# JohannesBuchner/UltraNest

Measured on AMD Instinct MI355X. Metric: proposal-points filtered/sec (MLFriends.inside) + region-rebuild ms, N=4000 d=50, higher is better.
Workload: dtype f64; 1 GPU; C5: N=4000 live points, d=50, P=1e6 proposals/step/GPU drawn uniformly inside the wrapping ellipsoid (set E), AffineLayer, 30 bootstraps; one step = MLFriends.inside on a batch resident in HBM; the timed loop visits 3 distinct batches in turn; n_live=4000, d=50, bootstraps=30, parallelism=proposal rows sharded over 1 GPU(s), region replicated

## Files before the change

ultranest_amd/csrc/mlf_filter.hpp:

```cpp
#pragma once
#include "mlf_common.hpp"
#include "mlf_prep4.hpp"

#define MLF_FILTER_MAXD 128

constexpr int kFilterMaxSplit = 16;

namespace mlf {

struct FilterArgs {
  const void *refF;
  const void *qF;
  const float *tlo, *thi;
  int ntiles32;
  long long ngroups;
  long long nq;
  int *best;
  unsigned long long *list;
  unsigned seg_cap;
  unsigned *seg_count;
  unsigned *counters;
  int tile0, tile1;
  const int *qmap;
  const unsigned *ngroups_dev;
  const unsigned *nslots_dev;
  int append;
  void *cq;
  float *ctlo, *cthi;
  int *cmap;
  unsigned *ccount;
  unsigned ccap;
  const uint8_t *route;
  long long seg_first_extra, seg_extra;
  int split;
  RecheckWArgs rw;
};
struct MinArgs {
  const void *refF;
  int ntiles32;
  int tile0, tile1;
  const void *qF;
  const float *tlo, *thi;
  const int *qmap;
  const int *qmin;
  long long ngroups;
  const unsigned *nslots_dev;
  long long nq;
  int *best;
  void *cq;
  float *ctlo, *cthi;
  int *cmap;
  int *cmin;
  unsigned *ccount;
  unsigned ccap;
  int last;
  unsigned long long *stamps;
  unsigned stamp_block;
};
constexpr unsigned kUncertainListCap = 4096;
struct UncertainArgs {
  const void *refF;
  int ntiles32;
  const void *qF;
  const float *thi;
  const int *qmap;
  const unsigned *nslots_dev;
  const double *pts;
  int d, dp;
  const double *lay_ctr;
  const double *T8;
  int ldt8;
  const double *refR;
  int n;
  double r2;
  int *best;
  unsigned *counters;
  unsigned *seg_count;
  EllExactArgs ell;
  unsigned nsweepblk;
};
hipError_t launch_sweep_min(int ks, int qw, const MinArgs &a, hipStream_t s);
hipError_t launch_uncertain(int ks, const UncertainArgs &a, hipStream_t s);
long long uncertain_blocks();
__host__ __device__ constexpr unsigned uncertain_stamp_base() { return 256u; }

struct MidArgs {
  const double *pts;
  long long np;
  int d, dp, ks;
  const void *LtF;
  const float *y0;
  const void *TtF;
  const double *lay_ctr;
  Prep4Consts c;
  const double *stats;
  double r2;
  const double *ell_ctr, *ell_L, *ell_A;
  double ell_eps_scale, enlarge;
  int chol_ok;
  const void *refF;
  int ntiles32;
  const double *refR;
  int n;
  const double *T64;
  unsigned long long *rec;
  unsigned long long *meta;
  unsigned *arrive;
  uint8_t *mask;
  uint8_t *route;
  unsigned *scan_flag;
  unsigned *counters;
  unsigned *stamps;
};
#define MLF_FOR_EACH_DP_MID(X)                                                                \
  X(2) X(4) X(6) X(8) X(10) X(12) X(14) X(16) X(18) X(20) X(22) X(24) X(26) X(28) X(30) X(32) \
  X(36) X(40) X(44) X(48) X(50) X(52) X(56)
bool mid_usable(int dp);
int mid_range_quads(long long ngroups, int ntiles32);
hipError_t launch_inside_mid(const MidArgs &a, int ny, hipStream_t s);

struct FusedArgs {
  Prep4Args p;
  const void *refF;
  int ntiles32;
  int tile0, tile1;
  void *cq;
  float *ctlo, *cthi;
  int *cmap, *cmin;
  unsigned *ccount;
  unsigned ccap;
  unsigned long long *stamps;
  unsigned stamp_block;
  unsigned variant;
};
bool fused_usable(int dp);
hipError_t launch_prep_sweep(const FusedArgs &a, hipStream_t s, int waves = 8);

void launch_phase_finish(void *cq, float *ctlo, float *cthi, int *cmap, unsigned *ccount, unsigned *ngroups_dst,
                         int ks, hipStream_t s);

struct RecheckArgs {
  const unsigned long long *list;
  unsigned seg_cap;
  const unsigned *seg_count;
  const double *refR;
  int n, d, dp;
  const double *q;
  long long ldq, ldk, nq;
  double r2;
  int *best;
};

void launch_ref_stats(const double *refR, int n, int d, int dp, double *stats, double *scratch, hipStream_t s,
                      unsigned long long *keys = nullptr);
void launch_quant_refs(const double *refR, int n, int npad32, int d, int dp, int ks,
                       const double *stats, void *refF, hipStream_t s, void *refFm = nullptr, const int *perm = nullptr,
                       double *rows_out = nullptr, int nrows_out = 0);
void launch_ref_rank(const unsigned long long *keys, int n, int *perm, hipStream_t s);
void launch_quant_queries(const double *q, long long ldq, long long nq, long long nqpad, int d_src, int d, int ks,
                          const double *stats, double r2, const uint8_t *gate, void *qF, float *tlo,
                          float *thi, uint8_t *route, int *best, unsigned *counters, hipStream_t s);
hipError_t launch_filter(int ks, const FilterArgs &a, bool first, hipStream_t s, int narrow = 0);
hipError_t launch_sweep(int ks, int qw, const FilterArgs &a, hipStream_t s);
int filter_groups_per_wave(int ks, int narrow);
void launch_recheck(const RecheckArgs &a, long long nwaves, hipStream_t s);
long long filter_wave_count(int ks, long long ngroups, int narrow = 0);
int filter_tile_split(int ks, long long ngroups, int ntiles, int target_waves = 2048);
void launch_filter_finalize(const uint8_t *route, const int *best, const unsigned *counters, long long nq,
                            uint8_t *out_mask, long long *out_idx, uint8_t *exact_gate, hipStream_t s,
                            unsigned *reset_word = nullptr);
void launch_route_gate(const uint8_t *route, const unsigned *counters, long long nq, int which,
                       uint8_t *gate, hipStream_t s);

}
```

ultranest_amd/csrc/mlf_sweepmin.hip:

```cpp
#include "mlf_filter.hpp"
#include "mlf_dpp_dev.hpp"
#include "mlf_filter_dev.hpp"
#include "mlf_recheck_dev.hpp"

#include <math.h>

namespace mlf {

typedef __attribute__((ext_vector_type(8))) _Float16 half8;
typedef __attribute__((ext_vector_type(16))) float float16v;
typedef __attribute__((ext_vector_type(4))) unsigned uint4v;

namespace {

__device__ __forceinline__ int min3i(int a, int b, int c) {
  const int m = a < b ? a : b;
  return m < c ? m : c;
}

constexpr int kPosInf = 0x7f800000;

template <int KS>
__device__ __forceinline__ void load_tile(half8 (&A)[KS], __amdgpu_buffer_rsrc_t rsrc, int voff, int soff) {
#pragma unroll
  for (int s = 0; s < KS; ++s) {
    union { uint4v u; half8 h; } c;
    c.u = __builtin_amdgcn_raw_buffer_load_b128(rsrc, voff, soff + s * 1024, 0);
    A[s] = c.h;
  }
}

__device__ __forceinline__ int tree_min(const float16v &c, int run) {
  const int m0 = min3i(__float_as_int(c[0]), __float_as_int(c[1]), __float_as_int(c[2]));
  const int m1 = min3i(__float_as_int(c[3]), __float_as_int(c[4]), __float_as_int(c[5]));
  const int m2 = min3i(__float_as_int(c[6]), __float_as_int(c[7]), __float_as_int(c[8]));
  const int m3 = min3i(__float_as_int(c[9]), __float_as_int(c[10]), __float_as_int(c[11]));
  const int m4 = min3i(__float_as_int(c[12]), __float_as_int(c[13]), __float_as_int(c[14]));
  return min3i(min3i(m0, m1, m2), min3i(m3, m4, __float_as_int(c[15])), run);
}

template <int I, int NM, int NV>
__device__ __forceinline__ void pin_step() {
  if constexpr (I < NM) {
    __builtin_amdgcn_sched_group_barrier(0x008, 1, 0);
    __builtin_amdgcn_sched_group_barrier(0x002, (NV * (I + 1)) / NM - (NV * I) / NM, 0);
    pin_step<I + 1, NM, NV>();
  }
}

__host__ __device__ constexpr int uncertain_row_stride(int d) { return d; }

__device__ __forceinline__ int uni(int v) { return __builtin_amdgcn_readfirstlane(v); }
__device__ __forceinline__ long long uni(long long v) {
  const unsigned lo = (unsigned)__builtin_amdgcn_readfirstlane((int)(unsigned)v);
  const unsigned hi = (unsigned)__builtin_amdgcn_readfirstlane((int)(unsigned)((unsigned long long)v >> 32));
  return (long long)(((unsigned long long)hi << 32) | lo);
}
template <class T>
__device__ __forceinline__ T *uni(T *p) {
  return reinterpret_cast<T *>(static_cast<uintptr_t>(uni((long long)reinterpret_cast<uintptr_t>(p))));
}

constexpr int min_waves(int ks, int qw, int pf) {
  const int need = 16 * qw + 4 * ks * qw + 4 * ks * (pf + 1) + 40;
  return (qw <= 2 && ks * qw <= 8) ? 4 : (need <= 128 ? 4 : (need <= 168 ? 3 : 2));
}

constexpr long long kSweepMinSetGrid = 1024;

}

template <int KS, int QW, int PF>
__global__ __launch_bounds__(256) __attribute__((amdgpu_waves_per_eu(min_waves(KS, QW, PF)))) void k_sweep_min(MinArgs a) {
  const int lane = threadIdx.x & 63;
  const long long nslots = a.nslots_dev ? (long long)*a.nslots_dev : -1;
  const long long ngroups = nslots >= 0 ? (nslots + 31) / 32 : a.ngroups;
  __shared__ unsigned wg_keep[4], wg_base;
  bool stamp_on = a.stamps != nullptr && blockIdx.x == a.stamp_block && threadIdx.x < 64;
  auto stamp = [&](int k) __attribute__((always_inline)) {
    if (stamp_on) {
      const unsigned long long t = __builtin_readcyclecounter();
      if (lane == 0) a.stamps[k] = t;
    }
  };
  stamp(0);
  auto stamp_rt = [&](int k) __attribute__((always_inline)) {
    if (a.stamps != nullptr && threadIdx.x == 0) {
      if (blockIdx.x == 0) a.stamps[8 + k] = __builtin_amdgcn_s_memrealtime();
      if (blockIdx.x == a.stamp_block) a.stamps[10 + k] = __builtin_amdgcn_s_memrealtime();
    }
  };
  stamp_rt(0);
  for (unsigned bidx = blockIdx.x, pass = 0;; bidx += gridDim.x, ++pass) {
  if ((long long)bidx * (4 * QW) >= ngroups) break;
  if (pass) __syncthreads();
  const long long wave = (long long)bidx * 4 + (threadIdx.x >> 6);
  const long long g0 = wave * QW;
  if (g0 >= ngroups) {
    if (lane == 0) wg_keep[threadIdx.x >> 6] = 0u;
    __syncthreads();
    __syncthreads();
    continue;
  }

  const half8 *qF = reinterpret_cast<const half8 *>(a.qF);
  half8 bq[QW][KS];
  float tlo[QW], thi[QW];
  int run[QW], qnum[QW];
#pragma unroll
  for (int g = 0; g < QW; ++g) {
    const long long grp = (g0 + g < ngroups) ? g0 + g : ngroups - 1;
#pragma unroll
    for (int s = 0; s < KS; ++s) bq[g][s] = qF[((size_t)grp * KS + s) * 64 + lane];
    const long long qi = grp * 32 + (lane & 31);
    const bool have = g0 + g < ngroups && (nslots < 0 || qi < nslots);
    tlo[g] = have ? a.tlo[qi] : -1.0f;
    thi[g] = have ? a.thi[qi] : -1.0f;
    if (!have) {
#pragma unroll
      for (int s = 0; s < KS; ++s) bq[g][s] = (half8){0, 0, 0, 0, 0, 0, 0, 0};
    }
    run[g] = (a.qmin && have && lane < 32) ? a.qmin[qi] : kPosInf;
    qnum[g] = have ? (a.qmap ? a.qmap[qi] : (int)qi) : -1;
  }

  const int ntl = a.tile1 - a.tile0;
  const int tstart = a.tile0 + (int)(((long long)bidx * 37) % ntl);
  constexpr int kTileBytes = KS * 1024;
  const __amdgpu_buffer_rsrc_t rsrc =
      __builtin_amdgcn_make_buffer_rsrc(const_cast<void *>(a.refF), 0, a.ntiles32 * kTileBytes, 0x00020000);
  const int voff = lane * 16;
  const int off_begin = a.tile0 * kTileBytes, off_end = a.tile1 * kTileBytes;

  float16v acc[QW];
  auto mm = [&](const half8(&A)[KS], int ga, int gb) __attribute__((always_inline)) {
#pragma unroll
    for (int s = 0; s < KS; ++s) {
      const float16v z = {0.f, 0.f, 0.f, 0.f, 0.f, 0.f, 0.f, 0.f, 0.f, 0.f, 0.f, 0.f, 0.f, 0.f, 0.f, 0.f};
      acc[ga] = __builtin_amdgcn_mfma_f32_32x32x16_f16(A[s], bq[ga][s], s == 0 ? z : acc[ga], 0, 0, 0);
      if (gb >= 0) acc[gb] = __builtin_amdgcn_mfma_f32_32x32x16_f16(A[s], bq[gb][s], s == 0 ? z : acc[gb], 0, 0, 0);
    }
  };
  auto next_off = [&](int off) __attribute__((always_inline)) {
    const int n = off + kTileBytes;
    return n == off_end ? off_begin : n;
  };
  auto tile = [&](const half8(&A)[KS]) __attribute__((always_inline)) {
    constexpr int NP = (QW + 1) / 2;
#pragma unroll
    for (int p = 0; p <= NP; ++p) {
      __builtin_amdgcn_sched_barrier(0);
      if (p < NP) mm(A, 2 * p, (2 * p + 1 < QW) ? 2 * p + 1 : -1);
      if (p > 0) {
#pragma unroll
        for (int g = 2 * (p - 1); g < 2 * p && g < QW; ++g) run[g] = tree_min(acc[g], run[g]);
      }
      if (NP == 2 && p == 1) pin_step<0, (QW == 4 ? 2 : 1) * KS, 16>();
    }
    __builtin_amdgcn_sched_barrier(0);
  };

  half8 A0[KS], A1[KS];
  if (PF == 2) {
    half8 A2[KS];
    int o0 = tstart * kTileBytes, o1 = next_off(o0), o2 = next_off(o1);
    load_tile<KS>(A0, rsrc, voff, o0);
    __builtin_amdgcn_sched_barrier(0);
    load_tile<KS>(A1, rsrc, voff, o1);
    __builtin_amdgcn_sched_barrier(0);
    stamp(1);
    for (int it = 0; it < ntl; it += 3) {
      load_tile<KS>(A2, rsrc, voff, o2);
      tile(A0);
      if (it == 0) stamp(2);
      if (it + 1 >= ntl) break;
      o0 = next_off(o2);
      load_tile<KS>(A0, rsrc, voff, o0);
      tile(A1);
      if (it + 2 >= ntl) break;
      o1 = next_off(o0);
      load_tile<KS>(A1, rsrc, voff, o1);
      tile(A2);
      o2 = next_off(o1);
    }
  } else {
    int off = tstart * kTileBytes;
    load_tile<KS>(A0, rsrc, voff, off);
    for (int it = 0; it < ntl; it += 2) {
      const int offn = next_off(off);
      load_tile<KS>(A1, rsrc, voff, offn);
      tile(A0);
      if (it + 1 >= ntl) break;
      off = next_off(offn);
      load_tile<KS>(A0, rsrc, voff, off);
      tile(A1);
    }
  }

  stamp(3);
  unsigned keepm[QW];
  int qid[QW], qmn[QW];
#pragma unroll
  for (int g = 0; g < QW; ++g) {
    keepm[g] = 0u;
    qid[g] = -1;
    qmn[g] = kPosInf;
    if (g0 + g >= ngroups) continue;
    const long long qi = qnum[g];
    const int m = half_min32(run[g]);
    const float mf = __int_as_float(m);
    const bool valid = qi >= 0 && qi < a.nq && thi[g] > 0.0f;
    const bool hit = valid && mf <= tlo[g];
    if (lane < 32 && hit) a.best[qi] = 0;
    const bool keep = valid && !hit && (a.last ? mf <= thi[g] : true);
    keepm[g] = (unsigned)__ballot(keep);
    qid[g] = (int)qi;
    qmn[g] = m;
  }
  unsigned total = 0;
#pragma unroll
  for (int g = 0; g < QW; ++g) total += (unsigned)__popc(keepm[g]);
  if (lane == 0) wg_keep[threadIdx.x >> 6] = total;
  stamp(4);
  __syncthreads();
  stamp(5);
  if (threadIdx.x == 0) {
    const unsigned all = wg_keep[0] + wg_keep[1] + wg_keep[2] + wg_keep[3];
    wg_base = all ? atomicAdd(a.ccount, all) : 0u;
  }
  __syncthreads();
  stamp(6);
  if (total != 0u) {
    unsigned base = wg_base;
    for (int w = 0; w < (int)(threadIdx.x >> 6); ++w) base += wg_keep[w];
    base = (unsigned)__builtin_amdgcn_readfirstlane((int)base);
    uint4 *dst = reinterpret_cast<uint4 *>(a.cq);
    const unsigned row = (unsigned)(lane & 31);
#pragma unroll
    for (int g = 0; g < QW; ++g) {
      if ((keepm[g] >> row) & 1u) {
        const unsigned rank = base + (unsigned)__popc(keepm[g] & ((1u << row) - 1u));
        const size_t gd = rank >> 5;
        const unsigned rd = (rank & 31u) + (unsigned)(lane & 32);
        if (rank < a.ccap) {
#pragma unroll
          for (int s = 0; s < KS; ++s) {
            union { half8 h; uint4 u; } cv;
            cv.h = bq[g][s];
            dst[(gd * KS + s) * 64 + rd] = cv.u;
          }
        }
        if (lane < 32 && rank < a.ccap) {
          a.ctlo[rank] = tlo[g];
          a.cthi[rank] = thi[g];
          a.cmap[rank] = qid[g];
          if (a.cmin) a.cmin[rank] = qmn[g];
        }
      }
      base += (unsigned)__popc(keepm[g]);
    }
  }
  stamp(7);
  if (stamp_on || (pass == 0 && blockIdx.x == 0)) stamp_rt(1);
  stamp_on = false;
  }
}

template <class T>
using lds_t = __attribute__((address_space(3))) T;
template <class T>
__device__ __forceinline__ lds_t<T> *lds_ptr(T *p) {
  return (lds_t<T> *)p;
}
template <class T>
__device__ __forceinline__ const lds_t<T> *lds_ptr(const T *p) {
  return (const lds_t<T> *)p;
}

template <int KS>
__device__ __attribute__((noinline)) void uncertain_sweep(const void *refF_, int ntiles32_, const void *qF_, const float *thi_, long long set_,
                                                          long long ngroups_, long long nslots_, unsigned *plist_, unsigned *lcount_,
                                                          int wv_, int lane) {
  constexpr int QW = 4;
  lds_t<unsigned> *plist = lds_ptr(plist_);
  lds_t<unsigned> *lcount = lds_ptr(lcount_);
  const void *refF = uni(refF_);
  const int ntiles32 = uni(ntiles32_), wv = uni(wv_);
  const long long set = uni(set_), ngroups = uni(ngroups_), nslots = uni(nslots_);
  qF_ = uni(qF_);
  thi_ = uni(thi_);
  typedef __attribute__((address_space(1))) const half8 ghalf8;
  typedef __attribute__((address_space(1))) const float gfloat;
  ghalf8 *qF = (ghalf8 *)qF_;
  gfloat *thig = (gfloat *)thi_;
  constexpr int kTileBytes = KS * 1024;
  const __amdgpu_buffer_rsrc_t rsrc =
      __builtin_amdgcn_make_buffer_rsrc(const_cast<void *>(refF), 0, ntiles32 * kTileBytes, 0x00020000);
  const int voff = lane * 16;
  const int rowbase = 4 * (lane >> 5);
  const long long g0 = set * QW;
  half8 bq[QW][KS];
  float thi[QW];
#pragma unroll
  for (int g = 0; g < QW; ++g) {
    const long long grp = (g0 + g < ngroups) ? g0 + g : ngroups - 1;
#pragma unroll
    for (int s = 0; s < KS; ++s) bq[g][s] = qF[((size_t)grp * KS + s) * 64 + lane];
    const long long qi = grp * 32 + (lane & 31);
    const bool have = g0 + g < ngroups && qi < nslots;
    thi[g] = have ? thig[qi] : -1.0f;
    if (!have) {
#pragma unroll
      for (int s = 0; s < KS; ++s) bq[g][s] = (half8){0, 0, 0, 0, 0, 0, 0, 0};
    }
  }
  const int tile0 = ntiles32 * wv / 8, tile1 = ntiles32 * (wv + 1) / 8;
  __builtin_amdgcn_s_waitcnt(0x0F70);
  float16v acc[QW];
  auto mm = [&](const half8(&A)[KS], int ga, int gb) __attribute__((always_inline)) {
#pragma unroll
    for (int s = 0; s < KS; ++s) {
      const float16v z = {0.f, 0.f, 0.f, 0.f, 0.f, 0.f, 0.f, 0.f, 0.f, 0.f, 0.f, 0.f, 0.f, 0.f, 0.f, 0.f};
      acc[ga] = __builtin_amdgcn_mfma_f32_32x32x16_f16(A[s], bq[ga][s], s == 0 ? z : acc[ga], 0, 0, 0);
      acc[gb] = __builtin_amdgcn_mfma_f32_32x32x16_f16(A[s], bq[gb][s], s == 0 ? z : acc[gb], 0, 0, 0);
    }
  };
  auto list_group = [&](int g, int t) __attribute__((always_inline)) {
    const float16v &c = acc[g];
    const int tm = tree_min(c, kPosInf);
    const bool flagged = __int_as_float(tm) <= thi[g];
    if (__ballot(flagged) == 0ull) return;
    unsigned bits = 0u;
    if (flagged) {
#pragma unroll
      for (int r = 0; r < 16; ++r) bits |= (c[r] <= thi[g]) ? (1u << r) : 0u;
    }
    if (bits != 0u) {
      unsigned at = __hip_atomic_fetch_add(lcount, (unsigned)__popc(bits), __ATOMIC_RELAXED, __HIP_MEMORY_SCOPE_WORKGROUP);
      const unsigned ql = (unsigned)(g * 32 + (lane & 31));
      while (bits != 0u) {
        const int r = __builtin_ctz(bits);
        bits &= bits - 1u;
        if (at < kUncertainListCap) plist[at] = (ql << 24) | (unsigned)(t * 32 + rowbase + (r & 3) + 8 * (r >> 2));
        ++at;
      }
    }
  };
  auto tile = [&](const half8(&A)[KS], int t) __attribute__((always_inline)) {
    mm(A, 0, 1);
    mm(A, 2, 3);
#pragma unroll
    for (int g = 0; g < QW; ++g) list_group(g, t);
  };
  half8 A0[KS], A1[KS], A2[KS];
  if (tile0 < tile1) {
    auto req = [&](half8(&A)[KS], int t) __attribute__((always_inline)) {
      load_tile<KS>(A, rsrc, voff, (t < tile1 ? t : tile1 - 1) * kTileBytes);
    };
    req(A0, tile0);
    __builtin_amdgcn_sched_barrier(0);
    req(A1, tile0 + 1);
    __builtin_amdgcn_sched_barrier(0);
    for (int t = tile0; t < tile1; t += 3) {
      req(A2, t + 2);
      tile(A0, t);
      if (t + 1 >= tile1) break;
      req(A0, t + 3);
      tile(A1, t + 1);
      if (t + 2 >= tile1) break;
      req(A1, t + 4);
      tile(A2, t + 2);
    }
  }
}

template <int NCH>
__device__ __attribute__((noinline)) void uncertain_pairs(const unsigned *plist_, unsigned cnt_, const int *qid_, const double *tq_,
                                                          const double *refR_, int dp_, int d_, int n_, double r2, int *best_) {
  const lds_t<unsigned> *plist = lds_ptr(plist_);
  const lds_t<int> *qid = lds_ptr(qid_);
  const lds_t<double> *tq = lds_ptr(tq_);
  typedef __attribute__((address_space(1))) const double gdouble;
  gdouble *refR = (gdouble *)uni(refR_);
  int *best = uni(best_);
  const int dp = uni(dp_), d = uni(d_), n = uni(n_);
  const unsigned cnt = (unsigned)uni((int)cnt_);
  const int ds = uncertain_row_stride(d);
  for (unsigned e = threadIdx.x; e < cnt; e += 512) {
    const unsigned ent = plist[e];
    const int ql = (int)(ent >> 24), i = (int)(ent & 0xffffffu);
    const int q = qid[ql];
    if (q < 0 || i >= n) continue;
    typedef double double2v __attribute__((ext_vector_type(2)));
    typedef __attribute__((address_space(1))) const double2v gdouble2;
    gdouble2 *ar = (gdouble2 *)(refR + (size_t)i * dp);
    const lds_t<double> *br = tq + ql * ds;
    double2v row[8 * NCH];
#pragma unroll
    for (int k2 = 0; k2 < 8 * NCH; ++k2) row[k2] = ar[k2];
    double accd = 0.0;
#pragma unroll
    for (int k2 = 0; k2 < 8 * NCH; ++k2) {
      const double d0 = row[k2].x - br[2 * k2];
      accd += 2 * k2 < d ? d0 * d0 : 0.0;
      const double d1 = row[k2].y - br[2 * k2 + 1];
      accd += 2 * k2 + 1 < d ? d1 * d1 : 0.0;
    }
    if (accd <= r2) atomicMin(&best[q], i);
  }
}

typedef double double4m __attribute__((ext_vector_type(4)));

template <int NK>
__device__ __attribute__((noinline)) void whiten16_mfma(const double *tl_, int ldt8_, int d_, int dp_, double *tq_, int wv_, int lane) {
  const lds_t<double> *tl = lds_ptr(tl_);
  lds_t<double> *tq = lds_ptr(tq_);
  const int ldt8 = uni(ldt8_), d = uni(d_), dp = uni(dp_), wv = uni(wv_);
  constexpr int NC = (NK + 3) / 4;
  const int ds = uncertain_row_stride(d);
  const int q = lane & 15, kq = lane >> 4;
  const lds_t<double> *row = tq + (16 * wv + q) * ds;
  double bfr[NK];
#pragma unroll
  for (int ks = 0; ks < NK; ++ks) {
    const int k = 4 * ks + kq;
    bfr[ks] = k < d ? row[k] : 0.0;
  }
  double4m t[NC];
#pragma unroll
  for (int ct = 0; ct < NC; ++ct) t[ct] = (double4m){0.0, 0.0, 0.0, 0.0};
#pragma unroll
  for (int ks = 0; ks < NK; ++ks) {
    const int k = 4 * ks + kq;
    double afr[NC];
#pragma unroll
    for (int ct = 0; ct < NC; ++ct) {
      const int c = 16 * ct + q;
      afr[ct] = (k < dp && c < d) ? tl[k * ldt8 + c] : 0.0;
    }
#pragma unroll
    for (int ct = 0; ct < NC; ++ct) t[ct] = __builtin_amdgcn_mfma_f64_16x16x4f64(afr[ct], bfr[ks], t[ct], 0, 0, 0);
  }
  __builtin_amdgcn_wave_barrier();
  lds_t<double> *out = tq + (16 * wv + q) * ds;
#pragma unroll
  for (int ct = 0; ct < NC; ++ct)
#pragma unroll
    for (int r = 0; r < 4; ++r) {
      const int c = 16 * ct + kq + 4 * r;
      if (c < d) out[c] = t[ct][r];
    }
}

template <int KS, int NCH>
__global__ __launch_bounds__(512, 1) void k_uncertain(UncertainArgs a) {
  constexpr int QW = 4;
  extern __shared__ __attribute__((aligned(16))) double lds_u[];
  const int lane = threadIdx.x & 63, wv = threadIdx.x >> 6;
  const int d = a.d, ds = uncertain_row_stride(d);
  double *tq = lds_u;
  double *tl = tq + 128 * ds;
  unsigned *plist = reinterpret_cast<unsigned *>(tl + a.dp * a.ldt8);
  int *qid = reinterpret_cast<int *>(plist + kUncertainListCap);
  unsigned *lcount = reinterpret_cast<unsigned *>(qid + 128);
  const unsigned nsweepblk = a.nsweepblk;
  if (blockIdx.x >= nsweepblk) {
    if (a.ell.count) ell_exact_wave(a.ell, lds_u + wv * 64, (blockIdx.x - nsweepblk) * 8 + wv, (gridDim.x - nsweepblk) * 8);
    return;
  }
  if (blockIdx.x == 0 && threadIdx.x == 0) {
#pragma unroll
    for (int k = 0; k < 8; ++k) a.seg_count[uncertain_stamp_base() + k] = 0u;
  }
  const long long nslots = (long long)*a.nslots_dev;
  if ((long long)blockIdx.x * 128 >= nslots) {
    if (threadIdx.x == 0) a.seg_count[blockIdx.x] = 0u;
    return;
  }
  unsigned nstamp = 0u;
  auto stamp = [&]() __attribute__((always_inline)) {
    if (blockIdx.x == 0 && threadIdx.x == 0 && nstamp < 8u) a.seg_count[uncertain_stamp_base() + nstamp] = (unsigned)__builtin_readcyclecounter();
    ++nstamp;
  };
  stamp();
  {
    double v[8];
    const int nt = a.dp * a.ldt8;
#pragma unroll
    for (int it = 0; it < 8; ++it) v[it] = threadIdx.x + it * 512 < nt ? a.T8[threadIdx.x + it * 512] : 0.0;
#pragma unroll
    for (int it = 0; it < 8; ++it)
      if (threadIdx.x + it * 512 < nt) tl[threadIdx.x + it * 512] = v[it];
  }
  const long long ngroups = (nslots + 31) / 32;
  const long long nsets = (ngroups + QW - 1) / QW;
  unsigned listed_total = 0u;

  for (long long set = blockIdx.x; set < nsets; set += nsweepblk) {
    __syncthreads();
    if (threadIdx.x == 0) *lcount = 0u;
    if (threadIdx.x < 128) {
      const long long slot = set * 128 + threadIdx.x;
      qid[threadIdx.x] = slot < nslots ? a.qmap[slot] : -1;
    }
    __syncthreads();
    stamp();
    uncertain_sweep<KS>(a.refF, a.ntiles32, a.qF, a.thi, set, ngroups, nslots, plist, lcount, wv, lane);
    stamp();
    {
      double v[16];
#pragma unroll
      for (int it = 0; it < 16; ++it) {
        const int e = threadIdx.x + it * 512;
        const int ql = e / d, k = e - ql * d;
        const int q = e < 128 * d ? qid[ql] : -1;
        v[it] = q >= 0 ? a.pts[(long long)q * d + k] - a.lay_ctr[k] : 0.0;
      }
#pragma unroll
      for (int it = 0; it < 16; ++it) {
        const int e = threadIdx.x + it * 512;
        const int ql = e / d, k = e - ql * d;
        if (e < 128 * d) tq[ql * ds + k] = v[it];
      }
    }
    __syncthreads();
    stamp();
    if (a.dp <= 16) whiten16_mfma<4>(tl, a.ldt8, d, a.dp, tq, wv, lane);
    else if (a.dp <= 32) whiten16_mfma<8>(tl, a.ldt8, d, a.dp, tq, wv, lane);
    else if (a.dp <= 52) whiten16_mfma<13>(tl, a.ldt8, d, a.dp, tq, wv, lane);
    else whiten16_mfma<16>(tl, a.ldt8, d, a.dp, tq, wv, lane);
    stamp();
    __syncthreads();
    stamp();
    const unsigned cnt = *lcount;
    if (cnt > kUncertainListCap) {
      if (threadIdx.x == 0) a.counters[1] = 1u;
    } else {
      uncertain_pairs<NCH>(plist, cnt, qid, tq, a.refR, a.dp, d, a.n, a.r2, a.best);
    }
    listed_total += cnt;
    stamp();
  }
  if (threadIdx.x == 0) a.seg_count[blockIdx.x] = listed_total;
}

template <int KS, int QW>
static hipError_t launch_sweep_min_t(const MinArgs &a, hipStream_t s) {
  const long long waves = (a.ngroups + QW - 1) / QW;
  long long wgs = (waves + 3) / 4;
  if (a.nslots_dev && wgs > kSweepMinSetGrid && wgs <= 2 * kSweepMinSetGrid) wgs = kSweepMinSetGrid;
  const dim3 grid((unsigned)wgs);
  constexpr int PF = (KS * QW >= 12 && KS <= 4) ? 2 : 1;
  hipLaunchKernelGGL((k_sweep_min<KS, QW, PF>), grid, dim3(256), 0, s, a);
  return hipGetLastError();
}

hipError_t launch_sweep_min(int ks, int qw, const MinArgs &a, hipStream_t s) {
  if (a.ngroups <= 0) return hipSuccess;
  switch (ks * 8 + qw) {
    case 1 * 8 + 4: return launch_sweep_min_t<1, 4>(a, s);
    case 2 * 8 + 4: return launch_sweep_min_t<2, 4>(a, s);
    case 3 * 8 + 4: return launch_sweep_min_t<3, 4>(a, s);
    case 4 * 8 + 4: return launch_sweep_min_t<4, 4>(a, s);
    case 1 * 8 + 2: return launch_sweep_min_t<1, 2>(a, s);
    case 2 * 8 + 2: return launch_sweep_min_t<2, 2>(a, s);
    case 3 * 8 + 2: return launch_sweep_min_t<3, 2>(a, s);
    case 4 * 8 + 2: return launch_sweep_min_t<4, 2>(a, s);
    default: return hipErrorInvalidValue;
  }
}

long long uncertain_blocks() { return 256; }

hipError_t launch_uncertain(int ks, const UncertainArgs &a_in, hipStream_t s) {
  UncertainArgs a = a_in;
  a.nsweepblk = (unsigned)uncertain_blocks();
  const dim3 grid(a.nsweepblk + (a.ell.count ? kEllWaves / 8 : 0u));
  const int ds = a.d | 1;
  const size_t lds = (size_t)128 * ds * sizeof(double) + (size_t)a.dp * a.ldt8 * sizeof(double) +
                     kUncertainListCap * sizeof(unsigned) + 128 * sizeof(int) + 16;
  const int nch = (a.dp + 15) / 16;
  if (a.dp > 64 || nch < 1) return hipErrorInvalidValue;
#define X(KS, NCH)                                                                                                          \
  if (ks == KS && nch == NCH) {                                                                                             \
    static DeviceGrant grant;                                                                                               \
    if (hipError_t e = grant.ensure([] {                                                                                    \
          return hipFuncSetAttribute(reinterpret_cast<const void *>(&k_uncertain<KS, NCH>),                                 \
                                     hipFuncAttributeMaxDynamicSharedMemorySize, 160 * 1024);                               \
        }))                                                                                                                 \
      return e;                                                                                                             \
    hipLaunchKernelGGL((k_uncertain<KS, NCH>), grid, dim3(512), lds, s, a);                                                 \
    return hipGetLastError();                                                                                               \
  }
  X(1, 1) X(2, 1) X(2, 2) X(3, 2) X(3, 3) X(4, 3) X(4, 4)
#undef X
  return hipErrorInvalidValue;
}

}
```

Baseline: 2.995 billion proposals/s.

## Shrink uncertain-kernel query sets to two groups to raise occupancy

Measured after the change: 3.017 billion proposals/s (median of 6 runs). Within noise of the previous version (+0.7%).

```diff
diff --git a/ultranest_amd/csrc/mlf_filter.hpp b/ultranest_amd/csrc/mlf_filter.hpp
--- a/ultranest_amd/csrc/mlf_filter.hpp
+++ b/ultranest_amd/csrc/mlf_filter.hpp
@@ -57,7 +57,14 @@
   unsigned long long *stamps;
   unsigned stamp_block;
 };
-constexpr unsigned kUncertainListCap = 4096;
+#ifndef MLF_UNCERTAIN_QW
+#define MLF_UNCERTAIN_QW 2
+#endif
+constexpr int kUncertainQW = MLF_UNCERTAIN_QW;
+static_assert(kUncertainQW == 2 || kUncertainQW == 4, "MLF_UNCERTAIN_QW: 2 or 4");
+constexpr unsigned kUncertainListCap = 1024u * kUncertainQW;
+constexpr unsigned kUncertainBlocks = kUncertainQW == 2 ? 512u : 256u;
+constexpr size_t kUncertainLdsMax = (kUncertainQW == 2 ? 80u : 160u) * 1024u;
 struct UncertainArgs {
   const void *refF;
   int ntiles32;
@@ -82,7 +89,7 @@
 hipError_t launch_sweep_min(int ks, int qw, const MinArgs &a, hipStream_t s);
 hipError_t launch_uncertain(int ks, const UncertainArgs &a, hipStream_t s);
 long long uncertain_blocks();
-__host__ __device__ constexpr unsigned uncertain_stamp_base() { return 256u; }
+__host__ __device__ constexpr unsigned uncertain_stamp_base() { return kUncertainBlocks; }
 
 struct MidArgs {
   const double *pts;
diff --git a/ultranest_amd/csrc/mlf_sweepmin.hip b/ultranest_amd/csrc/mlf_sweepmin.hip
--- a/ultranest_amd/csrc/mlf_sweepmin.hip
+++ b/ultranest_amd/csrc/mlf_sweepmin.hip
@@ -277,11 +277,11 @@
   return (const lds_t<T> *)p;
 }
 
-template <int KS>
+template <int KS, int QW>
 __device__ __attribute__((noinline)) void uncertain_sweep(const void *refF_, int ntiles32_, const void *qF_, const float *thi_, long long set_,
                                                           long long ngroups_, long long nslots_, unsigned *plist_, unsigned *lcount_,
                                                           int wv_, int lane) {
-  constexpr int QW = 4;
+  static_assert(QW == 2 || QW == 4, "a set is two or four 32-query groups");
   lds_t<unsigned> *plist = lds_ptr(plist_);
   lds_t<unsigned> *lcount = lds_ptr(lcount_);
   const void *refF = uni(refF_);
@@ -348,15 +348,30 @@
   };
   auto tile = [&](const half8(&A)[KS], int t) __attribute__((always_inline)) {
     mm(A, 0, 1);
-    mm(A, 2, 3);
+    if constexpr (QW == 4) mm(A, 2, 3);
 #pragma unroll
     for (int g = 0; g < QW; ++g) list_group(g, t);
   };
+  auto req = [&](half8(&A)[KS], int t) __attribute__((always_inline)) {
+    load_tile<KS>(A, rsrc, voff, (t < tile1 ? t : tile1 - 1) * kTileBytes);
+  };
+  if constexpr (QW == 2) {
+    half8 A0[KS], A1[KS];
+    if (tile0 < tile1) {
+      req(A0, tile0);
+      __builtin_amdgcn_sched_barrier(0);
+      for (int t = tile0; t < tile1; t += 2) {
+        req(A1, t + 1);
+        tile(A0, t);
+        if (t + 1 >= tile1) break;
+        req(A0, t + 2);
+        tile(A1, t + 1);
+      }
+    }
+    return;
+  }
   half8 A0[KS], A1[KS], A2[KS];
   if (tile0 < tile1) {
-    auto req = [&](half8(&A)[KS], int t) __attribute__((always_inline)) {
-      load_tile<KS>(A, rsrc, voff, (t < tile1 ? t : tile1 - 1) * kTileBytes);
-    };
     req(A0, tile0);
     __builtin_amdgcn_sched_barrier(0);
     req(A1, tile0 + 1);
@@ -395,18 +410,48 @@
     typedef __attribute__((address_space(1))) const double2v gdouble2;
     gdouble2 *ar = (gdouble2 *)(refR + (size_t)i * dp);
     const lds_t<double> *br = tq + ql * ds;
-    double2v row[8 * NCH];
-#pragma unroll
-    for (int k2 = 0; k2 < 8 * NCH; ++k2) row[k2] = ar[k2];
+    constexpr int H = 4 * NCH;
     double accd = 0.0;
 #pragma unroll
-    for (int k2 = 0; k2 < 8 * NCH; ++k2) {
-      const double d0 = row[k2].x - br[2 * k2];
-      accd += 2 * k2 < d ? d0 * d0 : 0.0;
-      const double d1 = row[k2].y - br[2 * k2 + 1];
-      accd += 2 * k2 + 1 < d ? d1 * d1 : 0.0;
+    for (int h = 0; h < 2; ++h) {
+      double2v row[H];
+#pragma unroll
+      for (int j = 0; j < H; ++j) row[j] = ar[h * H + j];
+#pragma unroll
+      for (int j = 0; j < H; ++j) {
+        const int k2 = h * H + j;
+        const double d0 = row[j].x - br[2 * k2];
+        accd += 2 * k2 < d ? d0 * d0 : 0.0;
+        const double d1 = row[j].y - br[2 * k2 + 1];
+        accd += 2 * k2 + 1 < d ? d1 * d1 : 0.0;
+      }
     }
     if (accd <= r2) atomicMin(&best[q], i);
+  }
+}
+
+template <int NQ>
+__device__ __attribute__((noinline)) void uncertain_rows(const double *pts_, const double *lay_ctr_, int d_, const int *qid_, double *tq_) {
+  typedef __attribute__((address_space(1))) const double gdouble;
+  gdouble *pts = (gdouble *)uni(pts_);
+  gdouble *lay_ctr = (gdouble *)uni(lay_ctr_);
+  const int d = uni(d_), ds = uncertain_row_stride(d);
+  const lds_t<int> *qid = lds_ptr(qid_);
+  lds_t<double> *tq = lds_ptr(tq_);
+  constexpr int NIT = NQ * 64 / 512;
+  double v[NIT];
+#pragma unroll
+  for (int it = 0; it < NIT; ++it) {
+    const int e = threadIdx.x + it * 512;
+    const int ql = e / d, k = e - ql * d;
+    const int q = e < NQ * d ? qid[ql] : -1;
+    v[it] = q >= 0 ? pts[(long long)q * d + k] - lay_ctr[k] : 0.0;
+  }
+#pragma unroll
+  for (int it = 0; it < NIT; ++it) {
+    const int e = threadIdx.x + it * 512;
+    const int ql = e / d, k = e - ql * d;
+    if (e < NQ * d) tq[ql * ds + k] = v[it];
   }
 }
 
@@ -453,17 +498,17 @@
     }
 }
 
-template <int KS, int NCH>
-__global__ __launch_bounds__(512, 1) void k_uncertain(UncertainArgs a) {
-  constexpr int QW = 4;
+template <int KS, int NCH, int QW = kUncertainQW>
+__global__ __launch_bounds__(512, QW == 2 ? 4 : 1) void k_uncertain(UncertainArgs a) {
+  constexpr int NQ = 32 * QW;
   extern __shared__ __attribute__((aligned(16))) double lds_u[];
-  const int lane = threadIdx.x & 63, wv = threadIdx.x >> 6;
+  const int lane = threadIdx.x & 63, wv = __builtin_amdgcn_readfirstlane(threadIdx.x >> 6);
   const int d = a.d, ds = uncertain_row_stride(d);
   double *tq = lds_u;
-  double *tl = tq + 128 * ds;
+  double *tl = tq + NQ * ds;
   unsigned *plist = reinterpret_cast<unsigned *>(tl + a.dp * a.ldt8);
   int *qid = reinterpret_cast<int *>(plist + kUncertainListCap);
-  unsigned *lcount = reinterpret_cast<unsigned *>(qid + 128);
+  unsigned *lcount = reinterpret_cast<unsigned *>(qid + NQ);
   const unsigned nsweepblk = a.nsweepblk;
   if (blockIdx.x >= nsweepblk) {
     if (a.ell.count) ell_exact_wave(a.ell, lds_u + wv * 64, (blockIdx.x - nsweepblk) * 8 + wv, (gridDim.x - nsweepblk) * 8);
@@ -474,7 +519,7 @@
     for (int k = 0; k < 8; ++k) a.seg_count[uncertain_stamp_base() + k] = 0u;
   }
   const long long nslots = (long long)*a.nslots_dev;
-  if ((long long)blockIdx.x * 128 >= nslots) {
+  if ((long long)blockIdx.x * NQ >= nslots) {
     if (threadIdx.x == 0) a.seg_count[blockIdx.x] = 0u;
     return;
   }
@@ -500,36 +545,23 @@
   for (long long set = blockIdx.x; set < nsets; set += nsweepblk) {
     __syncthreads();
     if (threadIdx.x == 0) *lcount = 0u;
-    if (threadIdx.x < 128) {
-      const long long slot = set * 128 + threadIdx.x;
+    if (threadIdx.x < NQ) {
+      const long long slot = set * NQ + threadIdx.x;
       qid[threadIdx.x] = slot < nslots ? a.qmap[slot] : -1;
     }
     __syncthreads();
     stamp();
-    uncertain_sweep<KS>(a.refF, a.ntiles32, a.qF, a.thi, set, ngroups, nslots, plist, lcount, wv, lane);
+    uncertain_sweep<KS, QW>(a.refF, a.ntiles32, a.qF, a.thi, set, ngroups, nslots, plist, lcount, wv, lane);
     stamp();
-    {
-      double v[16];
-#pragma unroll
-      for (int it = 0; it < 16; ++it) {
-        const int e = threadIdx.x + it * 512;
-        const int ql = e / d, k = e - ql * d;
-        const int q = e < 128 * d ? qid[ql] : -1;
-        v[it] = q >= 0 ? a.pts[(long long)q * d + k] - a.lay_ctr[k] : 0.0;
-      }
-#pragma unroll
-      for (int it = 0; it < 16; ++it) {
-        const int e = threadIdx.x + it * 512;
-        const int ql = e / d, k = e - ql * d;
-        if (e < 128 * d) tq[ql * ds + k] = v[it];
-      }
-    }
+    uncertain_rows<NQ>(a.pts, a.lay_ctr, d, qid, tq);
     __syncthreads();
     stamp();
-    if (a.dp <= 16) whiten16_mfma<4>(tl, a.ldt8, d, a.dp, tq, wv, lane);
-    else if (a.dp <= 32) whiten16_mfma<8>(tl, a.ldt8, d, a.dp, tq, wv, lane);
-    else if (a.dp <= 52) whiten16_mfma<13>(tl, a.ldt8, d, a.dp, tq, wv, lane);
-    else whiten16_mfma<16>(tl, a.ldt8, d, a.dp, tq, wv, lane);
+    if (wv < 2 * QW) {
+      if (a.dp <= 16) whiten16_mfma<4>(tl, a.ldt8, d, a.dp, tq, wv, lane);
+      else if (a.dp <= 32) whiten16_mfma<8>(tl, a.ldt8, d, a.dp, tq, wv, lane);
+      else if (a.dp <= 52) whiten16_mfma<13>(tl, a.ldt8, d, a.dp, tq, wv, lane);
+      else whiten16_mfma<16>(tl, a.ldt8, d, a.dp, tq, wv, lane);
+    }
     stamp();
     __syncthreads();
     stamp();
@@ -571,15 +603,17 @@
   }
 }
 
-long long uncertain_blocks() { return 256; }
+long long uncertain_blocks() { return kUncertainBlocks; }
 
 hipError_t launch_uncertain(int ks, const UncertainArgs &a_in, hipStream_t s) {
   UncertainArgs a = a_in;
   a.nsweepblk = (unsigned)uncertain_blocks();
   const dim3 grid(a.nsweepblk + (a.ell.count ? kEllWaves / 8 : 0u));
   const int ds = a.d | 1;
-  const size_t lds = (size_t)128 * ds * sizeof(double) + (size_t)a.dp * a.ldt8 * sizeof(double) +
-                     kUncertainListCap * sizeof(unsigned) + 128 * sizeof(int) + 16;
+  constexpr int NQ = 32 * kUncertainQW;
+  const size_t lds = (size_t)NQ * ds * sizeof(double) + (size_t)a.dp * a.ldt8 * sizeof(double) +
+                     kUncertainListCap * sizeof(unsigned) + NQ * sizeof(int) + 16;
+  if (lds > kUncertainLdsMax) return hipErrorInvalidValue;
   const int nch = (a.dp + 15) / 16;
   if (a.dp > 64 || nch < 1) return hipErrorInvalidValue;
 #define X(KS, NCH)                                                                                                          \
@@ -587,7 +621,7 @@
     static DeviceGrant grant;                                                                                               \
     if (hipError_t e = grant.ensure([] {                                                                                    \
           return hipFuncSetAttribute(reinterpret_cast<const void *>(&k_uncertain<KS, NCH>),                                 \
-                                     hipFuncAttributeMaxDynamicSharedMemorySize, 160 * 1024);                               \
+                                     hipFuncAttributeMaxDynamicSharedMemorySize, (int)kUncertainLdsMax);                                 \
         }))                                                                                                                 \
       return e;                                                                                                             \
     hipLaunchKernelGGL((k_uncertain<KS, NCH>), grid, dim3(512), lds, s, a);                                                 \
```
